# opencb/hpg-variant

Hardware: AMD Instinct MI355X
Metric: variants/s chi2 assoc (higher is better)
Workload: dtype u8

## Files before the change

hpg-variant_amd/csrc/hpgv_capi.hip:

```cpp
#include "hpgv_internal.h"
#include <cstdlib>

extern "C" {

const char *hpgv_version(void) { return "hpgv-mi355x 0.1 (gfx950)"; }

int hpgv_device_count(void) {
    int n = 0;
    if (hipGetDeviceCount(&n) != hipSuccess) return -1;
    return n;
}

const char *hpgv_last_error(const hpgv_ctx *ctx) { return ctx ? ctx->err.c_str() : g_create_error.c_str(); }

static void read_environment(hpgv_ctx *ctx) {
    auto num = [](const char *name, long lo, long hi, long *out) { const char *e = getenv(name); if (e && *e) { long v = atol(e); *out = v < lo ? lo : v > hi ? hi : v; } };
    num("HPGV_BATCH_COPY", 0, 1, &ctx->batch_copy);
    num("HPGV_BATCH_FUSED", 0, 1, &ctx->batch_fused);
    num("HPGV_STATS_ALL2", 0, 1, &ctx->stats_all2);
    num("HPGV_ASSOC_ROWS", 0, 1, &ctx->assoc_rows);
    num("HPGV_PINNED_NONCOHERENT", 0, 1, &ctx->pinned_noncoherent);
    num("HPGV_VMM_TRACE", 0, 1, &ctx->vmm_trace);
    num("HPGV_DECODE_TILES", 0, 1, &ctx->decode_tiles);
#ifdef HPGV_ABLATION
// ... 69 lines not shown
    g->device = g->members[0]->device;
    *out = g;
    return HPGV_OK;
}

int hpgv_group_size(const hpgv_ctx *ctx) { return !ctx ? 0 : (is_group(ctx) ? (int)ctx->members.size() : 1); }

hpgv_ctx *hpgv_group_member(hpgv_ctx *ctx, int i) {
    if (!ctx) return nullptr;
    if (!is_group(ctx)) return i == 0 ? ctx : nullptr;
    return (i >= 0 && i < (int)ctx->members.size()) ? ctx->members[(size_t)i] : nullptr;
}

int hpgv_member_device(const hpgv_ctx *ctx, int i) {
    if (!ctx) return -1;
    if (!is_group(ctx)) return i == 0 ? ctx->device : -1;
    return (i >= 0 && i < (int)ctx->members.size()) ? ctx->members[(size_t)i]->device : -1;
}

}
namespace {
void grow_release(hpgv_ctx::GrowRange &r) {
    size_t off = 0;
    for (size_t i = 0; i < r.pieces.size(); ++i) { (void)hipMemUnmap(r.base + off, r.sizes[i]); (void)hipMemRelease(r.pieces[i]); off += r.sizes[i]; }
    if (r.base) (void)hipMemAddressFree(r.base, r.reserved);
    r = hpgv_ctx::GrowRange();
}
}
extern "C" {

void hpgv_destroy(hpgv_ctx *ctx) {
    if (!ctx) return;
    if (is_group(ctx)) {
        hpgv_group_release(ctx);
        for (hpgv_ctx *m : ctx->members) { m->parent = nullptr; hpgv_destroy(m); }
        ctx->members.clear();
        delete ctx;
        return;
    }
    DeviceGuard g(ctx->device);
    (void)hipDeviceSynchronize();
    if (ctx->d_mendel_male) (void)hipFree(ctx->d_mendel_male);
    for (DevBuf *b : {&ctx->d_sg_chunks, &ctx->d_group_of_col, &ctx->d_cond, &ctx->d_perm, &ctx->d_strata, &ctx->d_cmh_tables, &ctx->d_cov, &ctx->d_lin, &ctx->d_linperm, &ctx->d_linperm_rows, &ctx->d_flips, &ctx->d_flip_tail, &ctx->d_thr, &ctx->assoc.d_cols, &ctx->tdt.d_cols,
                      &ctx->stats.d_cols, &ctx->sgroups.d_cols, &ctx->mendel.d_cols}) b->release();
    ctx->tdt_plan.release();
    if (ctx->d_lf_base) (void)hipFree(ctx->d_lf_base);
    if (ctx->d_sink) (void)hipFree(ctx->d_sink);
    if (ctx->d_crc_tab) (void)hipFree(ctx->d_crc_tab);
    for (auto *t : ctx->tok_scratch) {
        for (DevBuf *b : {&t->blocks, &t->line_off, &t->extra}) b->release();
        delete t;
    }
    ctx->tok_scratch.clear();
    for (auto &r : ctx->grow) grow_release(r);
    ctx->grow.clear();
    hpgv_epi_release(ctx->epi);
    for (Slot *s : ctx->slots) {
        s->release();
        if (s->stream) (void)hipStreamDestroy(s->stream);
        delete s;
    }
    for (int i = 0; i < 4; ++i) if (ctx->ev[i]) (void)hipEventDestroy(ctx->ev[i]);
    delete ctx;
}

#ifdef HPGV_ABLATION
#define HPGV_SHIPPED_ONLY(ok, what)
#else
#define HPGV_SHIPPED_ONLY(ok, what) if (!(ok)) return fail(ctx, HPGV_ERR_UNSUPPORTED, what ": that form is an ablation build's (-DHPGV_ABLATION, tools/build_ablation.py)");
#endif

int hpgv_set_option(hpgv_ctx *ctx, const char *key, long value) {
    if (is_group(ctx) && key && !strcmp(key, "group_self_exchange")) { ctx->group_self_exchange = value ? 1 : 0; return HPGV_OK; }
    if (is_group(ctx) && key && !strcmp(key, "group_fake_ranks")) {
        if (value < 0 || value > 65536) return fail(ctx, HPGV_ERR_INVALID, "group_fake_ranks must be 0 (ranks by distinct device) or the number of members that share rank 0");
        std::lock_guard<std::mutex> lk(ctx->mu);
        if (ctx->grp) return fail(ctx, HPGV_ERR_STATE, "group_fake_ranks must be set before the group's communicator exists (hpgv_group_comm_init, the first group call)");
        ctx->group_fake_ranks = value;
        return HPGV_OK;
    }
    GROUP_ALL(ctx, hpgv_set_option(m_, key, value))
    if (!ctx || !key) return HPGV_ERR_INVALID;
    if (!strcmp(key, "row_align")) {
        if (value < 16 || (value & (value - 1))) return fail(ctx, HPGV_ERR_INVALID, "row_align must be a power of two >= 16");
        if (ctx->assoc.set || ctx->tdt.set || ctx->stats.set)
            return fail(ctx, HPGV_ERR_STATE, "row_align must be set before the cohort");
        ctx->row_align = value;
    } else if (!strcmp(key, "row_pad")) {
        if (value < 0 || value % 16 || value > 65536) return fail(ctx, HPGV_ERR_INVALID, "row_pad must be a multiple of 16 in [0, 65536]");
        if (ctx->assoc.set || ctx->tdt.set || ctx->stats.set)
            return fail(ctx, HPGV_ERR_STATE, "row_pad must be set before the cohort");
        ctx->row_pad = value;
    } else if (!strcmp(key, "variants_per_wave")) {
        if (value < 1 || value > 1024) return fail(ctx, HPGV_ERR_INVALID, "variants_per_wave out of range");
        ctx->vpw = value;
    } else if (!strcmp(key, "nontemporal")) {
        HPGV_SHIPPED_ONLY(value != 0, "nontemporal = 0")
        ctx->nontemporal = value ? 1 : 0;
    } else if (!strcmp(key, "profile")) {
        ctx->profile = value ? 1 : 0;
    } else if (!strcmp(key, "scan_unroll")) {
        if (value != 4 && value != 8 && value != 10 && value != 12 && value != 16)
            return fail(ctx, HPGV_ERR_INVALID, "scan_unroll must be one of 4, 8, 10, 12, 16");
        HPGV_SHIPPED_ONLY(value == 4, "scan_unroll other than 4")
        ctx->scan_unroll = value;
    } else if (!strcmp(key, "pipeline")) {
        HPGV_SHIPPED_ONLY(value != 0, "pipeline = 0")
        ctx->pipeline = value ? 1 : 0;
    } else if (!strcmp(key, "fisher_cut_exp")) {
        if (value < 12 || value > 300) return fail(ctx, HPGV_ERR_INVALID, "fisher_cut_exp must be in [12, 300]");
        ctx->fisher_cut_exp = value;
    } else if (!strcmp(key, "epi_complete")) {
        ctx->epi_complete = value ? 1 : 0;
    } else if (!strcmp(key, "epi_triples_mfma")) {
        ctx->epi_triples_mfma = value ? 1 : 0;
    } else if (!strcmp(key, "epi_pairs_mfma")) {
        ctx->epi_pairs_mfma = value ? 1 : 0;
    } else if (!strcmp(key, "epi_wide")) {
        if (value < 0 || value > 2) return fail(ctx, HPGV_ERR_INVALID, "epi_wide must be 0 (the packed kernels' limits), 1 (the wide kernel where the shape needs it) or 2 (the wide kernel for every listed-combination launch)");
        ctx->epi_wide = value;
    } else if (!strcmp(key, "epi_triples_1pass")) {
        if (value < 0 || value > 2) return fail(ctx, HPGV_ERR_INVALID, "epi_triples_1pass must be 0 (two passes), 1 (the cells nine at a time) or 2 (one pass, one wave per SIMD)");
        HPGV_SHIPPED_ONLY(value != 2, "epi_triples_1pass = 2")
        ctx->epi_triples_1pass = value;
    } else if (!strcmp(key, "scan_lds")) {
        if (value < 0 || value > 160 * 1024) return fail(ctx, HPGV_ERR_INVALID, "scan_lds must be in [0, 163840]");
        ctx->scan_lds = value;
    } else if (!strcmp(key, "batch_copy")) {
        ctx->batch_copy = value ? 1 : 0;
    } else if (!strcmp(key, "inflate_wave")) {
        if (value < 0 || value > 4) return fail(ctx, HPGV_ERR_INVALID, "inflate_wave must be 0 (lane per block), 1 (by the number of blocks), 2 (wave per block), 4 (wave per block, several symbols per round) or 3 (lane per block, symbol tables in LDS)");
        HPGV_SHIPPED_ONLY(value == 1 || value == 4, "inflate_wave other than 1 / 4 (a wave per block, several symbols per round)")
        ctx->inflate_wave = value;
    } else if (!strcmp(key, "tokenizer_tiles")) {
        if (value < 0 || value > 2) return fail(ctx, HPGV_ERR_INVALID, "tokenizer_tiles must be 2 (one sweep), 1 (two sweeps) or 0 (line by line)");
        HPGV_SHIPPED_ONLY(value == 1, "tokenizer_tiles other than 1 (two sweeps)")
        ctx->tokenizer_tiles = value;
    } else if (!strcmp(key, "fisher_width")) {
        if (value != 64 && value != 32 && value != 16 && value != 8) return fail(ctx, HPGV_ERR_INVALID, "fisher_width must be 64, 32, 16 or 8");
        HPGV_SHIPPED_ONLY(value == 16, "fisher_width other than 16")
        ctx->fisher_width = value;
    } else if (!strcmp(key, "batch_fused")) {
        ctx->batch_fused = value ? 1 : 0;
    } else if (!strcmp(key, "pipe_waves")) {
        if (value != 4 && value != 6 && value != 8) return fail(ctx, HPGV_ERR_INVALID, "pipe_waves must be 4, 6 or 8");
        HPGV_SHIPPED_ONLY(value == 4, "pipe_waves other than 4")
        ctx->pipe_waves = value;
    } else if (!strcmp(key, "persistent")) {
        HPGV_SHIPPED_ONLY(value == 0, "persistent = 1")
        ctx->persistent = value ? 1 : 0;
    } else if (!strcmp(key, "part_aligned_loads")) {
        HPGV_SHIPPED_ONLY(value == 0, "part_aligned_loads = 1")
        ctx->part_aligned = value ? 1 : 0;
    } else if (!strcmp(key, "pca_apply_vector")) {
        HPGV_SHIPPED_ONLY(value == 0, "pca_apply_vector = 1")
        ctx->pca_apply_vector = value ? 1 : 0;
    } else if (!strcmp(key, "blocks_per_cu")) {
        if (value < 1 || value > 8) return fail(ctx, HPGV_ERR_INVALID, "blocks_per_cu must be in 1..8");
        ctx->blocks_per_cu = value;
    } else {
        return fail(ctx, HPGV_ERR_INVALID, "unknown option '%s'", key);
    }
    return HPGV_OK;
}


int hpgv_set_cohort(hpgv_ctx *ctx, const uint8_t *condition, int n_samples) {
    HPGV_ABI_TRY
    GROUP_ALL(ctx, hpgv_set_cohort(m_, condition, n_samples))
    if (!ctx) return HPGV_ERR_INVALID;
    if (!condition || n_samples < 0) return fail(ctx, HPGV_ERR_INVALID, "bad cohort arguments");
    DeviceGuard g(ctx->device);
    int nA = 0, nU = 0;
    for (int j = 0; j < n_samples; ++j) {
        if (condition[j] == HPGV_COND_AFFECTED) nA++;
        else if (condition[j] == HPGV_COND_UNAFFECTED) nU++;
    }
    size_t segA = round_up((size_t)nA, 16), segU = round_up((size_t)nU, 16);
    size_t pitch = round_up(segA + segU, (size_t)ctx->row_align) + (size_t)ctx->row_pad;
    if (pitch == 0) pitch = (size_t)ctx->row_align;
    if (!pitch_supported(pitch)) return fail(ctx, HPGV_ERR_UNSUPPORTED, "cohort of %d samples exceeds the row-length limit", n_samples);
    Layout &L = ctx->assoc;
    ctx->n_perms = ctx->perm_rows = 0;
    ctx->n_covar = 0;
    ctx->n_strata = ctx->strata_rows = 0;
    ctx->has_pheno = false; ctx->lin_y.clear(); ctx->lin_cov.clear();
    ctx->n_linperms = 0;
    L.n_samples = n_samples;
    L.pitch = pitch;
    L.col_of_pos.assign(pitch, -1);
    size_t a = 0, u = segA;
    for (int j = 0; j < n_samples; ++j) {
        if (condition[j] == HPGV_COND_AFFECTED) L.col_of_pos[a++] = j;
        else if (condition[j] == HPGV_COND_UNAFFECTED) L.col_of_pos[u++] = j;
    }
    ctx->nA = nA; ctx->nU = nU; ctx->chunksA = (int)(segA / 16);
    {
        std::vector<uint8_t> cond(round_up((size_t)n_samples, 16) + 16, (uint8_t)HPGV_COND_OTHER);
        for (int j = 0; j < n_samples; ++j) cond[(size_t)j] = condition[j] == HPGV_COND_AFFECTED ? 1 : condition[j] == HPGV_COND_UNAFFECTED ? 0 : 2;
        HIPCHK(ctx, ctx->d_cond.reserve(cond.size()));
        HIPCHK(ctx, hipMemcpy(ctx->d_cond.p, cond.data(), cond.size(), hipMemcpyHostToDevice));
    }
    return upload_layout(ctx, L);
    HPGV_ABI_CATCH(ctx)
}

int hpgv_assoc_layout(const hpgv_ctx *ctx, int *n_affected, int *n_unaffected, size_t *pitch) {
    ctx = first_member(ctx);
    if (!ctx) return HPGV_ERR_INVALID;
    if (!ctx->assoc.set) return fail(ctx, HPGV_ERR_STATE, "hpgv_set_cohort has not been called");
    if (n_affected) *n_affected = ctx->nA;
    if (n_unaffected) *n_unaffected = ctx->nU;
    if (pitch) *pitch = ctx->assoc.pitch;
    return HPGV_OK;
}

int hpgv_set_logfact(hpgv_ctx *ctx, const double *table, size_t n) {
    GROUP_ALL(ctx, hpgv_set_logfact(m_, table, n))
    if (!ctx) return HPGV_ERR_INVALID;
    if (!table || n == 0) return fail(ctx, HPGV_ERR_INVALID, "empty log-factorial table");
    DeviceGuard g(ctx->device);
    ctx->n_lf = 0;
    if (ctx->cap_lf < n) {
        if (ctx->d_lf_base) { (void)hipFree(ctx->d_lf_base); ctx->d_lf_base = nullptr; ctx->d_lf = nullptr; ctx->cap_lf = 0; }
        HIPCHK(ctx, hipMalloc(&ctx->d_lf_base, (n + 4) * sizeof(double)));
        HIPCHK(ctx, hipMemset(ctx->d_lf_base, 0, (n + 4) * sizeof(double)));
        ctx->d_lf = ctx->d_lf_base + 2;
        ctx->cap_lf = n;
    }
    HIPCHK(ctx, hipMemcpy(ctx->d_lf, table, n * sizeof(double), hipMemcpyHostToDevice));
    ctx->n_lf = n;
    return HPGV_OK;
}

int hpgv_set_stats_cohort(hpgv_ctx *ctx, int n_samples) {
    HPGV_ABI_TRY
    GROUP_ALL(ctx, hpgv_set_stats_cohort(m_, n_samples))
    if (!ctx) return HPGV_ERR_INVALID;
    if (n_samples < 0) return fail(ctx, HPGV_ERR_INVALID, "negative n_samples");
    DeviceGuard g(ctx->device);
    size_t pitch = round_up(round_up((size_t)n_samples, 16), (size_t)ctx->row_align);
    if (pitch == 0) pitch = (size_t)ctx->row_align;
    if (!pitch_supported(pitch)) return fail(ctx, HPGV_ERR_UNSUPPORTED, "cohort of %d samples exceeds the row-length limit", n_samples);
    Layout &L = ctx->stats;
    L.n_samples = n_samples;
    L.pitch = pitch;
    L.col_of_pos.assign(pitch, -1);
    for (int j = 0; j < n_samples; ++j) L.col_of_pos[j] = j;
    return upload_layout(ctx, L);
    HPGV_ABI_CATCH(ctx)
}

int hpgv_set_stats_groups(hpgv_ctx *ctx, const int32_t *group_of_sample, int n_samples, int n_groups) {
    HPGV_ABI_TRY
    GROUP_ALL(ctx, hpgv_set_stats_groups(m_, group_of_sample, n_samples, n_groups))
    if (!ctx) return HPGV_ERR_INVALID;
    if (n_samples < 0 || n_groups < 1 || n_groups > 4096 || (n_samples > 0 && !group_of_sample))
        return fail(ctx, HPGV_ERR_INVALID, "bad stats group arguments");
    DeviceGuard g(ctx->device);
    std::vector<int> size((size_t)n_groups, 0);
    for (int j = 0; j < n_samples; ++j) {
        if (group_of_sample[j] >= n_groups) return fail(ctx, HPGV_ERR_INVALID, "group %d of sample %d out of range", group_of_sample[j], j);
        if (group_of_sample[j] >= 0) size[(size_t)group_of_sample[j]]++;
    }
    std::vector<uint32_t> off((size_t)n_groups, 0);
    size_t used = 0;
    for (int k = 0; k < n_groups; ++k) { off[(size_t)k] = (uint32_t)used; used += round_up((size_t)size[(size_t)k], 16); }
    size_t pitch = round_up(used, (size_t)ctx->row_align) + (size_t)ctx->row_pad;
    if (pitch == 0) pitch = (size_t)ctx->row_align;
    if (!pitch_supported(pitch)) return fail(ctx, HPGV_ERR_UNSUPPORTED, "cohort of %d samples exceeds the row-length limit", n_samples);
    Layout &L = ctx->sgroups;
    L.n_samples = n_samples;
    L.pitch = pitch;
    L.col_of_pos.assign(pitch, -1);
    std::vector<size_t> fill(off.begin(), off.end());
    for (int j = 0; j < n_samples; ++j)
        if (group_of_sample[j] >= 0) L.col_of_pos[fill[(size_t)group_of_sample[j]]++] = j;
    ctx->sg_off = off;
    ctx->sg_size = size;
    {
// ... 369 lines not shown
```

hpg-variant_amd/csrc/hpgv_internal.h:

```cpp
#pragma once
#include "../../include/hpgv.h"
#include "hpgv_kernels.h"
#include "hpgv_tdt_stats_kernels.h"
#include "hpgv_epi_kernels.h"

#include <hip/hip_runtime.h>
#include <cctype>

#include <algorithm>
#include <atomic>
#include <cmath>
#include <cstdarg>
#include <cstdio>
#include <cstring>
#include <functional>
#include <mutex>
#include <new>
#include <string>
#include <vector>

namespace { thread_local std::string g_create_error; }

struct DevBuf {
    void *p = nullptr;
// ... 105 lines not shown
    uint32_t rev_off = 0;
    hpgv_epi_rank_info rank_info{};
    uint32_t *d_marg = nullptr;
    bool complete = false;
    hpgv::EpiChunk *d_chunks = nullptr;
    uint32_t *d_chunk_cls = nullptr;
    hpgv::EpiFold *d_folds = nullptr;
    uint32_t *d_group_w0 = nullptr;
    std::vector<int32_t> group_size;
    DevBuf cand;
    unsigned *d_cand_count = nullptr;
    unsigned cand_cap = 0;
    double *d_thr = nullptr;
    DevBuf tile_base;
};

struct hpgv_ctx {
    std::vector<hpgv_ctx *> members;
    hpgv_ctx *parent = nullptr;
    struct GroupState *grp = nullptr;
    long group_self_exchange = 0;
    long group_fake_ranks = 0;
    std::atomic<unsigned> deal_next{0};
    std::atomic<int> in_flight{0};
    int device = 0;
    mutable std::string err;
    std::mutex mu;
    long row_align = 16;
    long row_pad = 0;
    long vpw = 2;
    long nontemporal = 1;
    long profile = 0;
    std::mutex alias_mu;
    std::vector<std::pair<const char *, const char *>> text_alias;
    struct TextTiles { const char *d_text, *d_base; const void *d_tiles; uint64_t n_tiles; };
    std::vector<TextTiles> text_tiles;
    struct TextHeld { const char *host_text; Slot *slot; const char *d_text; const unsigned long long *d_line_off; int n_lines; };
    std::vector<TextHeld> text_held;
    long part_aligned = 0;
    long pca_apply_vector = 0;
    long scan_unroll = 4;
    long persistent = 0;
    long blocks_per_cu = 8;
    long pipeline = 1;
    long pipe_waves = 4;
    long fisher_cut_exp = 22;
    long epi_complete = 1;
    long epi_pairs_mfma = 1;
    long epi_triples_mfma = 1;
    long epi_wide = 0;
    long epi_triples_1pass = 1;
    long scan_lds = 0;
    long fisher_width = 16;
    long inflate_wave = 1;
    long tokenizer_tiles = 1;
    long batch_copy = 0;
    long batch_fused = 1;
    long batch_lds_max = 65536;
    long stats_all2 = 1;
    long assoc_rows = 1;
    long pinned_noncoherent = 0;
    long vmm_trace = 0;
    long decode_tiles = 1;
#ifdef HPGV_ABLATION
    long stats_rows = 0, stats_bs = 0, stats_debug = 0;
    long fisher_lds = 0;
    long inflate_lds_pad = 0, inflate_wave_wgs = 0, inflate_lane_wgs = 0;
#endif
    int n_cus = 256;
    Layout assoc;
    int nA = 0, nU = 0, chunksA = 0;
    DevBuf d_cond;
    DevBuf d_perm;
    int n_perms = 0, perm_rows = 0;
    DevBuf d_strata;
    int n_strata = 0, strata_rows = 0;
    DevBuf d_cmh_tables;
    DevBuf d_cov;
    int n_covar = 0;
    std::vector<double> lin_y, lin_cov;
    bool has_pheno = false;
    DevBuf d_lin;
    DevBuf d_linperm;
    int n_linperms = 0;
    DevBuf d_linperm_rows;
    Layout tdt;
    hpgv::TdtPlan tdt_plan;
    DevBuf d_flips;
    int n_flips = 0, flip_rows = 0, flip_pitch = 0;
    int tdt_families = 0;
    DevBuf d_flip_tail;
    Layout stats;
    Layout sgroups;
    std::vector<uint32_t> sg_off;
    std::vector<int> sg_size;
    DevBuf d_sg_chunks;
    DevBuf d_group_of_col;
    bool all_grouped = false;
    Layout mendel;
    int mendel_trios = 0, mendel_pchunks = 0;
    hpgv::MendelLuts mendel_luts{};
    uint8_t *d_mendel_male = nullptr;
    double *d_lf = nullptr;
    double *d_lf_base = nullptr;
    size_t n_lf = 0;
    size_t cap_lf = 0;
    DevBuf d_thr;
    hipEvent_t ev[4] = {nullptr, nullptr, nullptr, nullptr};
    bool have_scan_ev = false, have_stats_ev = false;
    std::vector<Slot *> slots;
    uint32_t *d_sink = nullptr;
    uint32_t *d_crc_tab = nullptr;
    struct TokScratch {
        hipStream_t stream = nullptr;
        DevBuf blocks, line_off, extra;
    };
    std::mutex tok_mu;
    std::vector<TokScratch *> tok_scratch;
    struct GrowRange { char *base = nullptr; size_t reserved = 0, committed = 0; std::vector<hipMemGenericAllocationHandle_t> pieces; std::vector<size_t> sizes; };
    std::vector<GrowRange> grow;
    double filt_min_maf = -1.0, filt_max_missing = -1.0;
    long filt_max_mendel = -1;
    double filt_min_dom = -1.0, filt_min_rec = -1.0;
    std::mutex epi_mu;
    EpiState epi;
};

namespace {

[[maybe_unused]] int fail(const hpgv_ctx *ctx, int code, const char *fmt, ...) {
    char buf[512];
    va_list ap;
    va_start(ap, fmt);
    vsnprintf(buf, sizeof buf, fmt, ap);
    va_end(ap);
    if (ctx) {
        ctx->err = buf;
        if (ctx->parent) {
            std::lock_guard<std::mutex> lk(ctx->parent->mu);
            ctx->parent->err = buf;
        }
    } else g_create_error = buf;
    return code;
}

#define HPGV_ABI_TRY try {
#define HPGV_ABI_CATCH(ctx)                                                                         \
    } catch (const std::bad_alloc &) { return fail(ctx, HPGV_ERR_NOMEM, "out of host memory"); }     \
      catch (...) { return fail(ctx, HPGV_ERR_INVALID, "unexpected C++ exception inside the engine"); }

inline bool is_group(const hpgv_ctx *c) { return c && !c->members.empty(); }
inline hpgv_ctx *first_member(hpgv_ctx *c) { return is_group(c) ? c->members[0] : c; }
inline const hpgv_ctx *first_member(const hpgv_ctx *c) { return is_group(c) ? c->members[0] : c; }
struct Dealt {
    hpgv_ctx *m;
    explicit Dealt(hpgv_ctx *g) {
        const unsigned n = (unsigned)g->members.size(), start = g->deal_next.fetch_add(1u, std::memory_order_relaxed) % n;
        m = g->members[start];
        int best = m->in_flight.load(std::memory_order_relaxed);
        for (unsigned k = 1; k < n && best > 0; ++k) {
            hpgv_ctx *c = g->members[(start + k) % n];
            const int f = c->in_flight.load(std::memory_order_relaxed);
            if (f < best) { best = f; m = c; }
        }
        m->in_flight.fetch_add(1, std::memory_order_relaxed);
    }
    ~Dealt() { m->in_flight.fetch_sub(1, std::memory_order_relaxed); }
};
#define GROUP_ALL(ctx, CALL)                                                                \
    if (is_group(ctx)) {                                                                    \
        for (hpgv_ctx *m_ : (ctx)->members) { const int rc_ = CALL; if (rc_) return rc_; }  \
// ... 199 lines not shown
```

hpg-variant_amd/csrc/hpgv_kernels.h:

```cpp
#pragma once
#include <hip/hip_runtime.h>
#include <stdint.h>

namespace hpgv {

__device__ __forceinline__ uint32_t nib_nonzero(uint32_t x) {
    uint32_t y = x | (x << 1);
    y = y | (y << 2);
    return y & 0x88888888u;
}
__device__ __forceinline__ uint32_t nib_not_f(uint32_t x) { return nib_nonzero(~x); }

__device__ __forceinline__ int wave_sum(int v) {
    v += __builtin_amdgcn_update_dpp(0, v, 0xB1, 0xF, 0xF, true);
    v += __builtin_amdgcn_update_dpp(0, v, 0x4E, 0xF, 0xF, true);
    v += __builtin_amdgcn_update_dpp(0, v, 0x141, 0xF, 0xF, true);
    v += __builtin_amdgcn_update_dpp(0, v, 0x140, 0xF, 0xF, true);
    return __builtin_amdgcn_readlane(v, 0) + __builtin_amdgcn_readlane(v, 16) +
           __builtin_amdgcn_readlane(v, 32) + __builtin_amdgcn_readlane(v, 48);
}

template <bool NT>
__device__ __forceinline__ uint4 load16(const uint4 *p);
template <bool NT>
// ... 219 lines not shown
    const int i = blockIdx.x * blockDim.x + threadIdx.x;
    if (i >= n) return;
    const int4 c4 = counts[i];
    const int a = c4.x, c = c4.y, b = c4.z, d = c4.w;
    const double x = assoc_chisq_value(a, c, b, d);
    odds[i] = assoc_odds(a, c, b, d);
    chisq[i] = x;
    pval[i] = chisq_p_value(x);
}

__device__ __forceinline__ double wave_sum_f64(double v) {
#pragma unroll
    for (int off = 32; off > 0; off >>= 1) v += __shfl_xor(v, off);
    return v;
}
__device__ __forceinline__ double wave_max_f64(double v) {
#pragma unroll
    for (int off = 32; off > 0; off >>= 1) { const double o = __shfl_xor(v, off); v = o > v ? o : v; }
    return v;
}

__device__ const double k_exp2_j64[64] = {
    0x1.0000000000000p+0, 0x1.02c9a3e778061p+0, 0x1.059b0d3158574p+0, 0x1.0874518759bc8p+0,
    0x1.0b5586cf9890fp+0, 0x1.0e3ec32d3d1a2p+0, 0x1.11301d0125b51p+0, 0x1.1429aaea92de0p+0,
    0x1.172b83c7d517bp+0, 0x1.1a35beb6fcb75p+0, 0x1.1d4873168b9aap+0, 0x1.2063b88628cd6p+0,
    0x1.2387a6e756238p+0, 0x1.26b4565e27cddp+0, 0x1.29e9df51fdee1p+0, 0x1.2d285a6e4030bp+0,
    0x1.306fe0a31b715p+0, 0x1.33c08b26416ffp+0, 0x1.371a7373aa9cbp+0, 0x1.3a7db34e59ff7p+0,
    0x1.3dea64c123422p+0, 0x1.4160a21f72e2ap+0, 0x1.44e086061892dp+0, 0x1.486a2b5c13cd0p+0,
    0x1.4bfdad5362a27p+0, 0x1.4f9b2769d2ca7p+0, 0x1.5342b569d4f82p+0, 0x1.56f4736b527dap+0,
    0x1.5ab07dd485429p+0, 0x1.5e76f15ad2148p+0, 0x1.6247eb03a5585p+0, 0x1.6623882552225p+0,
    0x1.6a09e667f3bcdp+0, 0x1.6dfb23c651a2fp+0, 0x1.71f75e8ec5f74p+0, 0x1.75feb564267c9p+0,
    0x1.7a11473eb0187p+0, 0x1.7e2f336cf4e62p+0, 0x1.82589994cce13p+0, 0x1.868d99b4492edp+0,
    0x1.8ace5422aa0dbp+0, 0x1.8f1ae99157736p+0, 0x1.93737b0cdc5e5p+0, 0x1.97d829fde4e50p+0,
    0x1.9c49182a3f090p+0, 0x1.a0c667b5de565p+0, 0x1.a5503b23e255dp+0, 0x1.a9e6b5579fdbfp+0,
    0x1.ae89f995ad3adp+0, 0x1.b33a2b84f15fbp+0, 0x1.b7f76f2fb5e47p+0, 0x1.bcc1e904bc1d2p+0,
    0x1.c199bdd85529cp+0, 0x1.c67f12e57d14bp+0, 0x1.cb720dcef9069p+0, 0x1.d072d4a07897cp+0,
    0x1.d5818dcfba487p+0, 0x1.da9e603db3285p+0, 0x1.dfc97337b9b5fp+0, 0x1.e502ee78b3ff6p+0,
    0x1.ea4afa2a490dap+0, 0x1.efa1bee615a27p+0, 0x1.f50765b6e4540p+0, 0x1.fa7c1819e90d8p+0,
};
__device__ __forceinline__ double fisher_exp(double e, const double *tab ) {
    const double kf = __builtin_rint(e * 0x1.71547652b82fep+6);
    double r = __builtin_fma(-kf, 0x1.62e42fe000000p-7, e);
    r = __builtin_fma(-kf, 0x1.f473de6af278fp-36, r);
    const int ki = (int)kf;
    const double tj = tab[ki & 63];
    double q = __builtin_fma(r, 1.0 / 120.0, 1.0 / 24.0);
    q = __builtin_fma(r, q, 1.0 / 6.0);
    q = __builtin_fma(r, q, 0.5);
    q = __builtin_fma(r * r, q, r);
    const double y = __builtin_fma(tj, q, tj);
    return e < -1100.0 ? 0.0 : __builtin_ldexp(y, ki >> 6);
}

struct FisherTab {
    const double *lf; const double *xt ; double konst; int r1, c1, d0;
    __device__ __forceinline__ double at(uint32_t byte_off) const { return *reinterpret_cast<const double *>(reinterpret_cast<const char *>(lf) + byte_off); }
    __device__ __forceinline__ double e(int x) const {
        const uint32_t x8 = (uint32_t)x << 3;
        return konst - at(x8) - at(((uint32_t)r1 << 3) - x8) - at(((uint32_t)c1 << 3) - x8) - at(((uint32_t)d0 << 3) + x8);
    }
    __device__ __forceinline__ double p(int x) const { return fisher_exp(e(x), xt); }
    __device__ __forceinline__ void e2(int x, double *e0, double *e1) const {
        const char *b = reinterpret_cast<const char *>(lf) - 16;
        double2 q0, q1, q2, q3;
        __builtin_memcpy(&q0, b + ((uint32_t)(x + 2) << 3), 16);
        __builtin_memcpy(&q1, b + ((uint32_t)(r1 - x + 1) << 3), 16);
        __builtin_memcpy(&q2, b + ((uint32_t)(c1 - x + 1) << 3), 16);
        __builtin_memcpy(&q3, b + ((uint32_t)(d0 + x + 2) << 3), 16);
        *e0 = konst - q0.x - q1.y - q2.y - q3.x;
        *e1 = konst - q0.y - q1.x - q2.x - q3.y;
    }
};

template <int W> __device__ __forceinline__ int sub_lane(int lane) { return lane & (W - 1); }
template <int W> __device__ __forceinline__ uint64_t sub_ballot(bool pred, int lane) {
    const uint64_t b = __ballot(pred);
    if constexpr (W == 64) { (void)lane; return b; }
    else return (b >> (lane & ~(W - 1))) & ((1ull << W) - 1ull);
}
template <int W> __device__ __forceinline__ double sub_sum_f64(double v) {
#pragma unroll
    for (int off = W / 2; off > 0; off >>= 1) v += __shfl_xor(v, off);
    return v;
}
template <int W> __device__ __forceinline__ double sub_first_f64(double v, int lane) { return __shfl(v, lane & ~(W - 1)); }

template <int W>
__device__ __forceinline__ void fisher_boundaries(const FisherTab &T, double thr , int L1, int R1, int L2, int R2, int lane,
                                                  int *xL, int *xR) {
    const int sl = sub_lane<W>(lane);
    while (R1 - L1 > W || R2 - L2 > W) {
        const bool go1 = R1 - L1 > W, go2 = R2 - L2 > W;
        const int step1 = (R1 - L1 + W - 1) / W, step2 = (R2 - L2 + W - 1) / W;
        const int x1 = L1 + sl * step1, x2 = L2 + sl * step2;
        const double v1 = (go1 && x1 < R1) ? T.e(x1) : 0.0;
        const double v2 = (go2 && x2 < R2) ? T.e(x2) : 0.0;
        if (go1) {
            const int j = __builtin_popcountll(sub_ballot<W>(x1 < R1 && v1 <= thr, lane));
            const int xj = L1 + j * step1;
            const int nL = (j == 0) ? L1 : L1 + (j - 1) * step1 + 1, nR = (j == W || xj >= R1) ? R1 : xj;
            L1 = nL; R1 = nR;
        }
        if (go2) {
            const int j = __builtin_popcountll(sub_ballot<W>(x2 < R2 && v2 > thr, lane));
            const int xj = L2 + j * step2;
            const int nL = (j == 0) ? L2 : L2 + (j - 1) * step2 + 1, nR = (j == W || xj >= R2) ? R2 : xj;
            L2 = nL; R2 = nR;
        }
    }
    const int x1 = L1 + sl, x2 = L2 + sl;
    const double v1 = x1 < R1 ? T.e(x1) : 0.0, v2 = x2 < R2 ? T.e(x2) : 0.0;
    *xL = L1 + __builtin_popcountll(sub_ballot<W>(x1 < R1 && v1 <= thr, lane));
    *xR = L2 + __builtin_popcountll(sub_ballot<W>(x2 < R2 && v2 > thr, lane));
}

template <int W>
__device__ __forceinline__ double fisher_tails(const FisherTab &T, int xL, int xR, int lo, int hi, int lane, double rel_cut) {
    const int sl = sub_lane<W>(lane);
    double partL = 0.0, partR = 0.0, cutL = 0.0, cutR = 0.0;
    bool onL = true, onR = true;
    for (int k = 0; onL || onR; ++k) {
        const int firstL = xL - 1 - 2 * W * k, firstR = xR + 2 * W * k;
        if (firstL < lo) onL = false;
// ... 45 lines not shown
    T.lf = lf; T.xt = exp_tab; T.r1 = r1; T.c1 = c1; T.d0 = r2 - c1;
    T.konst = lf[r1] + lf[r2] + lf[c1] + lf[nn - c1] - lf[nn];
    const double thr = T.e(a) + 9.9999995000000333e-08;
    double sum;
    if (hi - lo < 8 * W) {
        double part = 0.0;
        for (int x = lo + sl; x <= hi; x += W) {
            const double ex = T.e(x);
            if (ex <= thr) part += fisher_exp(ex, exp_tab);
        }
        sum = sub_sum_f64<W>(part);
    } else {
        const double prod = (double)(r1 + 1) * (double)(c1 + 1), den = (double)(nn + 2);
        double md = __builtin_floor(prod / den);
        const double rem = __builtin_fma(-md, den, prod);
        md += rem >= den ? 1.0 : (rem < 0.0 ? -1.0 : 0.0);
        int mode = (int)md;
        mode = mode < lo ? lo : (mode > hi ? hi : mode);
        int L1 = lo, R1 = mode + 1, L2 = mode + 1, R2 = hi + 1, xL, xR;
        if (fisher_boundary_windows<W>(T, thr, mode, a, lane, &L1, &R1, &L2, &R2)) { xL = L1; xR = L2; }
        else fisher_boundaries<W>(T, thr, L1, R1, L2, R2, lane, &xL, &xR);
        sum = fisher_tails<W>(T, xL, xR, lo, hi, lane, rel_cut);
    }
    return sum > 1.0 ? 1.0 : sum;
}

__device__ __forceinline__ double fisher_wave(int a, int b, int c, int d, const double *__restrict__ lf,
                                              const double *exp_tab , double rel_cut, int lane) {
    return fisher_sub<64>(a, b, c, d, lf, exp_tab, rel_cut, lane);
}

template <int W>
__global__ __launch_bounds__(256) void k_assoc_fisher(const int4 *__restrict__ counts, int n,
                                                      const double *__restrict__ lf,
                                                      double *__restrict__ odds,
                                                      double *__restrict__ pval, double rel_cut) {
    __shared__ double exp_tab[64];
    if (threadIdx.x < 64) exp_tab[threadIdx.x] = k_exp2_j64[threadIdx.x];
    __syncthreads();
    const int lane = threadIdx.x & 63;
    constexpr int PER_WAVE = 64 / W;
    const long wave = (long)blockIdx.x * (blockDim.x >> 6) + (threadIdx.x >> 6);
    const long v = wave * PER_WAVE + lane / W;
    if (v >= n) return;
    const int4 c4 = counts[v];
    const int a = c4.x, b = c4.y, c = c4.z, d = c4.w;
    const double p = fisher_sub<W>(a, b, c, d, lf, exp_tab, rel_cut, lane);
    if (sub_lane<W>(lane) == 0) {
        odds[v] = assoc_odds(a, b, c, d);
        pval[v] = p;
    }
}

__host__ __device__ __forceinline__ uint64_t splitmix64(uint64_t x) {
    x ^= x >> 30; x *= 0xbf58476d1ce4e5b9ULL;
    x ^= x >> 27; x *= 0x94d049bb133111ebULL;
    x ^= x >> 31;
    return x;
}
#define HPGV_SYNTH_SEED 0x4850475631ULL

static __global__ void k_synth_thresholds(uint64_t v0, int n, uint32_t *__restrict__ thr) {
    const int i = blockIdx.x * blockDim.x + threadIdx.x;
    if (i >= n) return;
    const uint64_t v = v0 + (uint64_t)i;
    const uint64_t h = splitmix64(HPGV_SYNTH_SEED ^ 0xA11E1EULL ^ v);
    const double u = (double)(h >> 11) * (1.0 / 9007199254740992.0);
    const double q = 0.05 + 0.45 * u;
    const uint32_t t_miss = 167772u;
    const double rest = (double)(16777216u - t_miss);
    const double omq = 1.0 - q;
    const double p00 = omq * omq;
    const double p01 = 2.0 * q * omq;
    const uint32_t t00 = t_miss + (uint32_t)floor(p00 * rest);
    const uint32_t t01 = t00 + (uint32_t)floor(p01 * rest);
    thr[3 * i + 0] = t_miss; thr[3 * i + 1] = t00; thr[3 * i + 2] = t01;
}

__device__ __forceinline__ uint32_t synth_gt(uint64_t vterm, uint64_t s, uint32_t tm, uint32_t t0,
                                             uint32_t t1) {
    const uint32_t r = (uint32_t)(splitmix64(vterm + s) >> 40);
    return (r < tm) ? 0xFFu : (r < t0) ? 0x00u : (r < t1) ? 0x01u : 0x11u;
}

enum { RECODE_NONE = 0, RECODE_TDT = 1, RECODE_STATS = 2, RECODE_MENDEL = 3, RECODE_EPI = 4 };

constexpr uint32_t TDT_F_UNUSABLE = 0x80u, TDT_M_UNUSABLE = 0x20u;
constexpr uint32_t TDT_C_INVALID = 4u;

__host__ __device__ __forceinline__ uint32_t tdt_parent_class(uint32_t g, uint32_t unusable) {
    const uint32_t a1 = g >> 4, a2 = g & 0xFu;
    if (a1 == 0xFu || a2 == 0xFu) return unusable;
    if (a1 && !a2) return unusable;
    if (!a1 && !a2) return 0u;
    if (!a1) return 1u;
    return (a1 == a2) ? 2u : 3u;
}
__host__ __device__ __forceinline__ uint32_t tdt_child_class(uint32_t g) {
    const uint32_t a1 = g >> 4, a2 = g & 0xFu;
    if (a1 == 0xFu || a2 == 0xFu) return TDT_C_INVALID;
    if (!a1 && !a2) return 0u;
    if (!a1) return 1u;
    if (!a2) return 2u;
    return 3u;
}
__host__ __device__ __forceinline__ uint32_t stats_flags(uint32_t g) {
// ... 139 lines not shown
```

hpg-variant_amd/csrc/hpgv_scan_capi.hip:

```cpp
#include "hpgv_internal.h"
#include <type_traits>
#include "hpgv_inherit_kernels.h"

namespace {

unsigned scan_blocks(const hpgv_ctx *ctx, int n_variants) {
    const long waves = ((long)n_variants + ctx->vpw - 1) / ctx->vpw;
    return (unsigned)((waves + 3) / 4);
}

const char *const kAligned16 = "device buffers must be 16-byte aligned";
int scan_checks(hpgv_ctx *ctx, int n_variants, const void *d_gt, const void *d_out, uintptr_t out_mask, const char *align_text, bool *go) {
    *go = false;
    if (n_variants < 0 || (n_variants > 0 && (!d_gt || !d_out))) return fail(ctx, HPGV_ERR_INVALID, "bad scan arguments");
    if (n_variants == 0) return HPGV_OK;
    if (((uintptr_t)d_gt & 15) || ((uintptr_t)d_out & out_mask)) return fail(ctx, HPGV_ERR_INVALID, "%s", align_text);
    *go = true;
    return HPGV_OK;
}

template <typename F>
void launch_nt(const hpgv_ctx *ctx, F &&f) {
    if (ctx->nontemporal) f(std::true_type{}); else f(std::false_type{});
}
// ... 152 lines not shown
    do {                                                                                         \
        if (ctx->pipe_waves == 8) { HPGV_LAUNCH_PIPE(NT, U, 8); }                                \
        else if (ctx->pipe_waves == 6) { HPGV_LAUNCH_PIPE(NT, U, 6); }                           \
        else { HPGV_LAUNCH_PIPE(NT, U, 4); }                                                     \
    } while (0)
    if (ctx->pipeline && !ctx->persistent)
        return launch_profiled(ctx, st, 0, [&] {
            if (ctx->nontemporal) {
                if (ctx->scan_unroll <= 4) HPGV_PIPE_W(true, 4); else HPGV_PIPE_W(true, 5);
            } else {
                if (ctx->scan_unroll <= 4) HPGV_PIPE_W(false, 4); else HPGV_PIPE_W(false, 5);
            }
        });
    return launch_profiled(ctx, st, 0, [&] {
        if (ctx->nontemporal) {
            if (ctx->persistent) { HPGV_DISPATCH_U(true, true) } else { HPGV_DISPATCH_U(true, false) }
        } else {
            if (ctx->persistent) { HPGV_DISPATCH_U(false, true) } else { HPGV_DISPATCH_U(false, false) }
        }
    });
#undef HPGV_DISPATCH_U
#undef HPGV_PIPE_W
#undef HPGV_LAUNCH_ASSOC
#endif
#undef HPGV_LAUNCH_PIPE
}

int hpgv_assoc_chisq_dev(hpgv_ctx *ctx, const int32_t *d_counts, int n_variants, double *d_odds,
                         double *d_chisq, double *d_p, void *stream) {
    ctx = first_member(ctx);
    if (!ctx) return HPGV_ERR_INVALID;
    if (n_variants < 0 || (n_variants > 0 && (!d_counts || !d_odds || !d_chisq || !d_p)))
        return fail(ctx, HPGV_ERR_INVALID, "bad chisq arguments");
    if (n_variants == 0) return HPGV_OK;
    DeviceGuard g(ctx->device);
    hipStream_t st = (hipStream_t)stream;
    return launch_profiled(ctx, st, 1, [&] {
        hipLaunchKernelGGL(hpgv::k_assoc_chisq, dim3((n_variants + 255) / 256), dim3(256), 0, st,
                           (const int4 *)d_counts, n_variants, d_odds, d_chisq, d_p);
    });
}

int hpgv_assoc_fisher_dev(hpgv_ctx *ctx, const int32_t *d_counts, int n_variants, double *d_odds,
                          double *d_p, void *stream) {
    ctx = first_member(ctx);
    if (!ctx) return HPGV_ERR_INVALID;
    if (n_variants < 0 || (n_variants > 0 && (!d_counts || !d_odds || !d_p)))
        return fail(ctx, HPGV_ERR_INVALID, "bad fisher arguments");
    if (const int rc = logfact_check(ctx)) return rc;
    if (n_variants == 0) return HPGV_OK;
    DeviceGuard g(ctx->device);
    hipStream_t st = (hipStream_t)stream;
    const double cut = pow(10.0, -(double)ctx->fisher_cut_exp);
    return launch_profiled(ctx, st, 1, [&] {
        const long per_block = 4 * (64 / ctx->fisher_width);
        const unsigned blocks = (unsigned)(((long)n_variants + per_block - 1) / per_block);
#ifdef HPGV_ABLATION
        const unsigned pad = (unsigned)ctx->fisher_lds;
        if (ctx->fisher_width == 64)
            hipLaunchKernelGGL(hpgv::k_assoc_fisher<64>, dim3(blocks), dim3(256), pad, st, (const int4 *)d_counts, n_variants, ctx->d_lf, d_odds, d_p, cut);
        else if (ctx->fisher_width == 8)
            hipLaunchKernelGGL(hpgv::k_assoc_fisher<8>, dim3(blocks), dim3(256), pad, st, (const int4 *)d_counts, n_variants, ctx->d_lf, d_odds, d_p, cut);
        else if (ctx->fisher_width == 32)
            hipLaunchKernelGGL(hpgv::k_assoc_fisher<32>, dim3(blocks), dim3(256), pad, st, (const int4 *)d_counts, n_variants, ctx->d_lf, d_odds, d_p, cut);
        else
#else
        const unsigned pad = 0u;
#endif
            hipLaunchKernelGGL(hpgv::k_assoc_fisher<16>, dim3(blocks), dim3(256), pad, st, (const int4 *)d_counts, n_variants, ctx->d_lf, d_odds, d_p, cut);
    });
}


int hpgv_tdt_scan_dev(hpgv_ctx *ctx, const uint8_t *d_gt, int n_variants, const uint8_t *d_is_x,
                      int32_t *d_tu, void *stream) {
    ctx = first_member(ctx);
    if (!ctx) return HPGV_ERR_INVALID;
    if (!ctx->tdt.set) return fail(ctx, HPGV_ERR_STATE, "hpgv_set_families has not been called");
    bool go;
    if (const int rc = scan_checks(ctx, n_variants, d_gt, d_tu, 7, "device buffers must be aligned", &go); rc || !go) return rc;
    DeviceGuard g(ctx->device);
    hipStream_t st = (hipStream_t)stream;
    return launch_profiled(ctx, st, 0, [&] {
        ctx->tdt_plan.launch_scan(d_gt, ctx->tdt.pitch, n_variants, d_is_x, (int2 *)d_tu,
                                  (int)ctx->vpw, ctx->nontemporal != 0, st);
    });
}

int hpgv_tdt_stats_dev(hpgv_ctx *ctx, const int32_t *d_tu, int n_variants, double *d_odds,
                       double *d_chisq, double *d_p, void *stream) {
    ctx = first_member(ctx);
    if (!ctx) return HPGV_ERR_INVALID;
    if (n_variants < 0 || (n_variants > 0 && (!d_tu || !d_odds || !d_chisq || !d_p)))
        return fail(ctx, HPGV_ERR_INVALID, "bad tdt stats arguments");
    if (n_variants == 0) return HPGV_OK;
    DeviceGuard g(ctx->device);
    hipStream_t st = (hipStream_t)stream;
    return launch_profiled(ctx, st, 1, [&] {
        hipLaunchKernelGGL(hpgv::k_tdt_stats, dim3((n_variants + 255) / 256), dim3(256), 0, st,
                           (const int2 *)d_tu, n_variants, d_odds, d_chisq, d_p);
    });
}


static int stats_scan(hpgv_ctx *ctx, const Layout &L, const uint8_t *d_gt, int n_variants, uint32_t off, int chunks, size_t lds,
                      int32_t *d_counts8, hipStream_t st) {
// ... 198 lines not shown
```

Before: 136.1 million.

## Split Fisher exact test into plan, scan and load-balanced sum kernels

For large Fisher calls, a plan kernel locates each variant's tail ranges with Newton steps and galloping search, then counts 32-term chunks. A prefix scan over those counts lets a persistent sum kernel give every 16-lane group an equal share of chunks. This is meant to remove the load imbalance from variants with very different tail lengths. It adds two extra launches, a per-stream scratch buffer, and a larger zero pad on the log-factorial table.

New measurement: 135.8 million, median of 2. No clear change (-0.2%).

```diff
diff --git a/hpg-variant_amd/csrc/hpgv_capi.hip b/hpg-variant_amd/csrc/hpgv_capi.hip
--- a/hpg-variant_amd/csrc/hpgv_capi.hip
+++ b/hpg-variant_amd/csrc/hpgv_capi.hip
@@ -145,6 +145,8 @@
         delete t;
     }
     ctx->tok_scratch.clear();
+    for (auto *t : ctx->fisher_scratch) { t->buf.release(); delete t; }
+    ctx->fisher_scratch.clear();
     for (auto &r : ctx->grow) grow_release(r);
     ctx->grow.clear();
     hpgv_epi_release(ctx->epi);
@@ -233,6 +235,9 @@
         if (value != 64 && value != 32 && value != 16 && value != 8) return fail(ctx, HPGV_ERR_INVALID, "fisher_width must be 64, 32, 16 or 8");
         HPGV_SHIPPED_ONLY(value == 16, "fisher_width other than 16")
         ctx->fisher_width = value;
+    } else if (!strcmp(key, "fisher_dense_min")) {
+        if (value < 0) return fail(ctx, HPGV_ERR_INVALID, "fisher_dense_min must be 0 (every call in two phases) or a number of variants");
+        ctx->fisher_dense_min = value;
     } else if (!strcmp(key, "batch_fused")) {
         ctx->batch_fused = value ? 1 : 0;
     } else if (!strcmp(key, "pipe_waves")) {
@@ -316,9 +321,9 @@
     ctx->n_lf = 0;
     if (ctx->cap_lf < n) {
         if (ctx->d_lf_base) { (void)hipFree(ctx->d_lf_base); ctx->d_lf_base = nullptr; ctx->d_lf = nullptr; ctx->cap_lf = 0; }
-        HIPCHK(ctx, hipMalloc(&ctx->d_lf_base, (n + 4) * sizeof(double)));
-        HIPCHK(ctx, hipMemset(ctx->d_lf_base, 0, (n + 4) * sizeof(double)));
-        ctx->d_lf = ctx->d_lf_base + 2;
+        HIPCHK(ctx, hipMalloc(&ctx->d_lf_base, (n + 2 * hpgv::FISHER_LF_PAD) * sizeof(double)));
+        HIPCHK(ctx, hipMemset(ctx->d_lf_base, 0, (n + 2 * hpgv::FISHER_LF_PAD) * sizeof(double)));
+        ctx->d_lf = ctx->d_lf_base + hpgv::FISHER_LF_PAD;
         ctx->cap_lf = n;
     }
     HIPCHK(ctx, hipMemcpy(ctx->d_lf, table, n * sizeof(double), hipMemcpyHostToDevice));
diff --git a/hpg-variant_amd/csrc/hpgv_internal.h b/hpg-variant_amd/csrc/hpgv_internal.h
--- a/hpg-variant_amd/csrc/hpgv_internal.h
+++ b/hpg-variant_amd/csrc/hpgv_internal.h
@@ -181,6 +181,7 @@
     long epi_triples_1pass = 1;
     long scan_lds = 0;
     long fisher_width = 16;
+    long fisher_dense_min = 524288;
     long inflate_wave = 1;
     long tokenizer_tiles = 1;
     long batch_copy = 0;
@@ -246,6 +247,12 @@
     };
     std::mutex tok_mu;
     std::vector<TokScratch *> tok_scratch;
+    struct FisherScratch {
+        hipStream_t stream = nullptr;
+        DevBuf buf;
+    };
+    std::vector<FisherScratch *> fisher_scratch;
+    int fisher_sum_blocks = 0;
     struct GrowRange { char *base = nullptr; size_t reserved = 0, committed = 0; std::vector<hipMemGenericAllocationHandle_t> pieces; std::vector<size_t> sizes; };
     std::vector<GrowRange> grow;
     double filt_min_maf = -1.0, filt_max_missing = -1.0;
diff --git a/hpg-variant_amd/csrc/hpgv_kernels.h b/hpg-variant_amd/csrc/hpgv_kernels.h
--- a/hpg-variant_amd/csrc/hpgv_kernels.h
+++ b/hpg-variant_amd/csrc/hpgv_kernels.h
@@ -295,6 +295,7 @@
     return e < -1100.0 ? 0.0 : __builtin_ldexp(y, ki >> 6);
 }
 
+constexpr int FISHER_LF_PAD = 40;
 struct FisherTab {
     const double *lf; const double *xt ; double konst; int r1, c1, d0;
     __device__ __forceinline__ double at(uint32_t byte_off) const { return *reinterpret_cast<const double *>(reinterpret_cast<const char *>(lf) + byte_off); }
@@ -303,15 +304,24 @@
         return konst - at(x8) - at(((uint32_t)r1 << 3) - x8) - at(((uint32_t)c1 << 3) - x8) - at(((uint32_t)d0 << 3) + x8);
     }
     __device__ __forceinline__ double p(int x) const { return fisher_exp(e(x), xt); }
-    __device__ __forceinline__ void e2(int x, double *e0, double *e1) const {
-        const char *b = reinterpret_cast<const char *>(lf) - 16;
+    __device__ __forceinline__ void e2_at(uint32_t o0, uint32_t o1, uint32_t o2, uint32_t o3, double *e0, double *e1) const {
+        const char *b = reinterpret_cast<const char *>(lf) - 8 * FISHER_LF_PAD;
         double2 q0, q1, q2, q3;
-        __builtin_memcpy(&q0, b + ((uint32_t)(x + 2) << 3), 16);
-        __builtin_memcpy(&q1, b + ((uint32_t)(r1 - x + 1) << 3), 16);
-        __builtin_memcpy(&q2, b + ((uint32_t)(c1 - x + 1) << 3), 16);
-        __builtin_memcpy(&q3, b + ((uint32_t)(d0 + x + 2) << 3), 16);
+        __builtin_memcpy(&q0, b + o0, 16);
+        __builtin_memcpy(&q1, b + o1, 16);
+        __builtin_memcpy(&q2, b + o2, 16);
+        __builtin_memcpy(&q3, b + o3, 16);
         *e0 = konst - q0.x - q1.y - q2.y - q3.x;
         *e1 = konst - q0.y - q1.x - q2.x - q3.y;
+    }
+    __device__ __forceinline__ void offsets(int x, uint32_t *o0, uint32_t *o1, uint32_t *o2, uint32_t *o3) const {
+        *o0 = (uint32_t)(x + FISHER_LF_PAD) << 3; *o1 = (uint32_t)(r1 - x - 1 + FISHER_LF_PAD) << 3;
+        *o2 = (uint32_t)(c1 - x - 1 + FISHER_LF_PAD) << 3; *o3 = (uint32_t)(d0 + x + FISHER_LF_PAD) << 3;
+    }
+    __device__ __forceinline__ void e2(int x, double *e0, double *e1) const {
+        uint32_t o0, o1, o2, o3;
+        offsets(x, &o0, &o1, &o2, &o3);
+        e2_at(o0, o1, o2, o3, e0, e1);
     }
 };
 
@@ -463,6 +473,214 @@
     }
 }
 
+struct FisherPlan { double konst, thr; int pos1, end1, pos2, end2; };
+constexpr int FISHER_CHUNK = 32;
+constexpr int FISHER_PLAN_BLOCK = 256;
+__host__ __device__ constexpr unsigned fisher_chunks(int pos1, int end1, int pos2, int end2) {
+    const unsigned c = (unsigned)(end1 - pos1 + FISHER_CHUNK - 1) / FISHER_CHUNK + (unsigned)(end2 - pos2 + FISHER_CHUNK - 1) / FISHER_CHUNK;
+    return c ? c : 1u;
+}
+
+template <typename P>
+__device__ __forceinline__ int fisher_count_true(P pred, int N, int guess) {
+    if (N <= 0) return 0;
+    int L = 0, R = N, s = 1;
+    const int g = guess < 0 ? 0 : (guess > N - 1 ? N - 1 : guess);
+    if (pred(g)) {
+        L = g + 1;
+        while (L < R) { const int x = (R - L > s) ? L + s - 1 : R - 1; if (pred(x)) { L = x + 1; s *= 4; } else { R = x; break; } }
+    } else {
+        R = g;
+        while (L < R) { const int x = (R - L > s) ? R - s : L; if (!pred(x)) { R = x; s *= 4; } else { L = x + 1; break; } }
+    }
+    while (L < R) { const int m = L + ((R - L) >> 1); if (pred(m)) L = m + 1; else R = m; }
+    return L;
+}
+__device__ __forceinline__ int fisher_newton(const FisherTab &T, int x, double target, int xmin, int xmax) {
+    x = x < xmin ? xmin : (x > xmax ? xmax : x);
+    const float num = (float)(T.r1 - x) * (float)(T.c1 - x), den = (float)(x + 1) * (float)(T.d0 + x + 1);
+    const float dx = (float)(target - T.e(x)) / __logf(num / den);
+    if (!(__builtin_fabsf(dx) < 1e6f)) return x;
+    const int y = x + (int)__builtin_rintf(dx);
+    return y < xmin ? xmin : (y > xmax ? xmax : y);
+}
+
+__device__ __forceinline__ int fisher_tail_end(const FisherTab &T, int x, double cutline, int xmin, int xmax, int dir) {
+    x = x < xmin ? xmin : (x > xmax ? xmax : x);
+#pragma unroll 1
+    for (int k = 0; k < 2; ++k) {
+        const float num = (float)(T.r1 - x) * (float)(T.c1 - x), den = (float)(x + 1) * (float)(T.d0 + x + 1);
+        const float dx = (float)(cutline - T.e(x)) / __logf(num / den);
+        if (!(__builtin_fabsf(dx) < 1e6f)) return dir > 0 ? xmax : xmin;
+        const int y = x + (int)(dir > 0 ? __builtin_ceilf(dx) : __builtin_floorf(dx)) + dir;
+        const int moved = y > x ? y - x : x - y;
+        x = y < xmin ? xmin : (y > xmax ? xmax : y);
+        if (moved <= 8) break;
+    }
+    return x;
+}
+
+static __global__ __launch_bounds__(FISHER_PLAN_BLOCK) void k_assoc_fisher_plan(const int4 *__restrict__ counts, int n, const double *__restrict__ lf,
+                                                                          double ln_cut, FisherPlan *__restrict__ plan,
+                                                                          double *__restrict__ odds, uint32_t *__restrict__ local_start,
+                                                                          uint32_t *__restrict__ block_sum) {
+    __shared__ uint32_t wave_tot[FISHER_PLAN_BLOCK / 64];
+    const long v = (long)blockIdx.x * FISHER_PLAN_BLOCK + threadIdx.x;
+    uint32_t chunks = 0;
+    if (v < n) {
+        const int4 c4 = counts[v];
+        const int a = c4.x, b = c4.y, c = c4.z, d = c4.w;
+        const int r1 = a + b, r2 = c + d, c1 = a + c, nn = r1 + r2;
+        const int lo = (c1 - r2) > 0 ? (c1 - r2) : 0;
+        const int hi = r1 < c1 ? r1 : c1;
+        FisherTab T;
+        T.lf = lf; T.xt = nullptr; T.r1 = r1; T.c1 = c1; T.d0 = r2 - c1;
+        T.konst = lf[r1] + lf[r2] + lf[c1] + lf[nn - c1] - lf[nn];
+        const double thr = T.e(a) + 9.9999995000000333e-08;
+        FisherPlan P;
+        P.konst = T.konst;
+        if (hi - lo < 8 * 16) {
+            P.thr = thr; P.pos1 = lo; P.end1 = hi + 1; P.pos2 = P.end2 = lo;
+        } else {
+            const double prod = (double)(r1 + 1) * (double)(c1 + 1), den = (double)(nn + 2);
+            double md = __builtin_floor(prod / den);
+            const double rem = __builtin_fma(-md, den, prod);
+            md += rem >= den ? 1.0 : (rem < 0.0 ? -1.0 : 0.0);
+            int mode = (int)md;
+            mode = mode < lo ? lo : (mode > hi ? hi : mode);
+            const bool left = a <= mode;
+            int gL = left ? a + 1 : 2 * mode - a + 1, gR = left ? 2 * mode - a : a;
+            if (left) { if (hi > mode) gR = fisher_newton(T, gR, thr, mode + 1, hi); }
+            else gL = fisher_newton(T, gL, thr, lo, mode);
+            double e_firstL = 0.0, e_firstR = 0.0;
+            const int xL = lo + fisher_count_true([&](int i) { const double ex = T.e(lo + i); const bool in = ex <= thr; if (in) e_firstL = ex; return in; },
+                                                  mode + 1 - lo, gL - lo);
+            const int xR = mode + 1 + fisher_count_true([&](int i) { const double ex = T.e(mode + 1 + i); const bool out = ex > thr; if (!out) e_firstR = ex; return out; },
+                                                        hi - mode, gR - (mode + 1));
+            const float fn = (float)nn, var2 = 2.0f * (float)r1 * (float)r2 / fn * (float)c1 / fn * (float)(nn - c1) / (fn > 1.0f ? fn - 1.0f : 1.0f);
+            int lenL = 0, lenR = 0;
+            if (xL > lo) {
+                const int first = xL - 1;
+                const float z = (float)(mode - first);
+                const int end = fisher_tail_end(T, first - (int)(__builtin_sqrtf(z * z - var2 * (float)ln_cut) - __builtin_fabsf(z)), e_firstL + ln_cut, lo, first, -1);
+                lenL = first - end + 1;
+            }
+            if (xR <= hi) {
+                const float z = (float)(xR - mode);
+                const int end = fisher_tail_end(T, xR + (int)(__builtin_sqrtf(z * z - var2 * (float)ln_cut) - __builtin_fabsf(z)), e_firstR + ln_cut, xR, hi, 1);
+                lenR = end - xR + 1;
+            }
+            P.thr = __builtin_huge_val(); P.pos1 = xL - lenL; P.end1 = xL; P.pos2 = xR; P.end2 = xR + lenR;
+        }
+        plan[v] = P;
+        odds[v] = assoc_odds(a, b, c, d);
+        chunks = fisher_chunks(P.pos1, P.end1, P.pos2, P.end2);
+    }
+    const int lane = threadIdx.x & 63, wave = threadIdx.x >> 6;
+    uint32_t incl = chunks;
+#pragma unroll
+    for (int off = 1; off < 64; off <<= 1) { const uint32_t o = __shfl_up(incl, off); if (lane >= off) incl += o; }
+    if (lane == 63) wave_tot[wave] = incl;
+    __syncthreads();
+    uint32_t before = 0, all = 0;
+#pragma unroll
+    for (int w = 0; w < FISHER_PLAN_BLOCK / 64; ++w) { const uint32_t t = wave_tot[w]; all += t; if (w < wave) before += t; }
+    if (v < n) local_start[v] = before + incl - chunks;
+    if (threadIdx.x == 0) block_sum[blockIdx.x] = all;
+}
+
+static __global__ __launch_bounds__(1024) void k_assoc_fisher_offsets(const uint32_t *__restrict__ block_sum, int nb, unsigned long long *__restrict__ block_off) {
+    __shared__ unsigned long long s[1024];
+    const int tid = threadIdx.x, per = (nb + 1023) / 1024;
+    const long b0 = (long)tid * per, b1 = b0 + per < nb ? b0 + per : nb;
+    unsigned long long sum = 0;
+    for (long i = b0; i < b1; ++i) sum += block_sum[i];
+    s[tid] = sum;
+    __syncthreads();
+    for (int off = 1; off < 1024; off <<= 1) {
+        const unsigned long long t = tid >= off ? s[tid - off] : 0ull;
+        __syncthreads();
+        s[tid] += t;
+        __syncthreads();
+    }
+    unsigned long long run = s[tid] - sum;
+    for (long i = b0; i < b1; ++i) { block_off[i] = run; run += block_sum[i]; }
+    if (tid == 1023) block_off[nb] = s[1023];
+}
+
+__device__ __forceinline__ double row16_sum_f64(double v) {
+#define HPGV_ROW_STEP(ctrl)                                                                                  \
+    {                                                                                                        \
+        const int l_ = __builtin_amdgcn_update_dpp(0, __double2loint(v), ctrl, 0xF, 0xF, false);            \
+        const int h_ = __builtin_amdgcn_update_dpp(0, __double2hiint(v), ctrl, 0xF, 0xF, false);            \
+        v += __hiloint2double(h_, l_);                                                                       \
+    }
+    HPGV_ROW_STEP(0xB1)
+    HPGV_ROW_STEP(0x4E)
+    HPGV_ROW_STEP(0x141)
+    HPGV_ROW_STEP(0x140)
+#undef HPGV_ROW_STEP
+    return v;
+}
+
+static __global__ __launch_bounds__(256) void k_assoc_fisher_sum(const FisherPlan *__restrict__ plan, const int4 *__restrict__ counts,
+                                                                 const uint32_t *__restrict__ local_start,
+                                                                 const unsigned long long *__restrict__ block_off, int n,
+                                                                 const double *__restrict__ lf, double *__restrict__ pval) {
+    __shared__ double exp_tab[64];
+    if (threadIdx.x < 64) exp_tab[threadIdx.x] = k_exp2_j64[threadIdx.x];
+    __syncthreads();
+    const int sl2 = 2 * (threadIdx.x & 15);
+    const unsigned long long G = (unsigned long long)gridDim.x * 16, g = (unsigned long long)blockIdx.x * 16 + (threadIdx.x >> 4);
+    const unsigned long long total = block_off[(n + FISHER_PLAN_BLOCK - 1) / FISHER_PLAN_BLOCK], Q = (total + G - 1) / G;
+    auto start_of = [&](int vv) { return vv < n ? block_off[vv / FISHER_PLAN_BLOCK] + local_start[vv] : total; };
+    auto first_at = [&](unsigned long long key) {
+        int L = 0, R = n;
+        while (L < R) {
+            const int step = (R - L + 15) >> 4, m = L + (sl2 >> 1) * step;
+            const int j = __builtin_popcountll(sub_ballot<16>(m < R && start_of(m) < key, threadIdx.x & 63));
+            if (j == 0) R = L;
+            else { const int mj = L + j * step; R = (j < 16 && mj < R) ? mj : R; L = L + (j - 1) * step + 1; }
+        }
+        return L;
+    };
+    int v = first_at(g * Q);
+    const int vend = first_at((g + 1) * Q);
+    const int n_chunks = (int)(start_of(vend) - start_of(v));
+    FisherTab T;
+    T.lf = lf; T.xt = exp_tab;
+    double thr = 0.0, part = 0.0;
+    int rem = 0, pos2 = 0, end2 = 0;
+    uint32_t o0 = 0, o1 = 0, o2 = 0, o3 = 0;
+    auto range = [&](int pos, int end) { T.offsets(pos + sl2, &o0, &o1, &o2, &o3); rem = end - pos - sl2; };
+    auto load = [&](int vv) {
+        const FisherPlan P = plan[vv];
+        const int4 c4 = counts[vv];
+        T.konst = P.konst; T.r1 = c4.x + c4.y; T.c1 = c4.x + c4.z; T.d0 = c4.w - c4.x;
+        thr = P.thr; pos2 = P.pos2; end2 = P.end2;
+        if (P.pos1 < P.end1) range(P.pos1, P.end1);
+        else { range(pos2, end2); pos2 = end2; }
+    };
+    auto masked = [](double t, bool in) { return __hiloint2double(in ? __double2hiint(t) : (int)0xC09F4000, __double2loint(t)); };
+    if (n_chunks > 0) load(v);
+    for (int c = 0; c < n_chunks; ++c) {
+        double t0, t1;
+        T.e2_at(o0, o1, o2, o3, &t0, &t1);
+        const double e0 = masked(t0, rem > 0 && t0 <= thr), e1 = masked(t1, rem > 1 && t1 <= thr);
+        part += fisher_exp(e0, exp_tab) + fisher_exp(e1, exp_tab);
+        o0 += 8 * FISHER_CHUNK; o1 -= 8 * FISHER_CHUNK; o2 -= 8 * FISHER_CHUNK; o3 += 8 * FISHER_CHUNK; rem -= FISHER_CHUNK;
+        if (rem + sl2 <= 0) {
+            if (pos2 < end2) { range(pos2, end2); pos2 = end2; }
+            else {
+                const double sum = row16_sum_f64(part);
+                if (sl2 == 0) pval[v] = sum > 1.0 ? 1.0 : sum;
+                part = 0.0;
+                if (++v < vend) load(v);
+            }
+        }
+    }
+}
+
 __host__ __device__ __forceinline__ uint64_t splitmix64(uint64_t x) {
     x ^= x >> 30; x *= 0xbf58476d1ce4e5b9ULL;
     x ^= x >> 27; x *= 0x94d049bb133111ebULL;
diff --git a/hpg-variant_amd/csrc/hpgv_scan_capi.hip b/hpg-variant_amd/csrc/hpgv_scan_capi.hip
--- a/hpg-variant_amd/csrc/hpgv_scan_capi.hip
+++ b/hpg-variant_amd/csrc/hpgv_scan_capi.hip
@@ -228,6 +228,36 @@
     DeviceGuard g(ctx->device);
     hipStream_t st = (hipStream_t)stream;
     const double cut = pow(10.0, -(double)ctx->fisher_cut_exp);
+    if (ctx->fisher_width == 16 && n_variants >= ctx->fisher_dense_min) {
+        hpgv_ctx::FisherScratch *fs = nullptr;
+        {
+            std::lock_guard<std::mutex> lk(ctx->tok_mu);
+            for (auto *t : ctx->fisher_scratch) if (t->stream == st) fs = t;
+            if (!fs) { fs = new hpgv_ctx::FisherScratch(); fs->stream = st; ctx->fisher_scratch.push_back(fs); }
+            if (!ctx->fisher_sum_blocks) {
+                int per_cu = 0;
+                HIPCHK(ctx, hipOccupancyMaxActiveBlocksPerMultiprocessor(&per_cu, hpgv::k_assoc_fisher_sum, 256, 0));
+                ctx->fisher_sum_blocks = (per_cu > 0 ? per_cu : 1) * ctx->n_cus;
+            }
+        }
+        const size_t n = (size_t)n_variants, nb = (n + hpgv::FISHER_PLAN_BLOCK - 1) / hpgv::FISHER_PLAN_BLOCK;
+        const size_t off_boff = n * sizeof(hpgv::FisherPlan), off_local = off_boff + round_up((nb + 1) * sizeof(unsigned long long), 16),
+                     off_bsum = off_local + round_up(n * sizeof(uint32_t), 16), bytes = off_bsum + nb * sizeof(uint32_t);
+        HIPCHK(ctx, fs->buf.reserve_after_sync(st, bytes, bytes + bytes / 4));
+        char *base = fs->buf.as<char>();
+        hpgv::FisherPlan *plan = (hpgv::FisherPlan *)base;
+        unsigned long long *boff = (unsigned long long *)(base + off_boff);
+        uint32_t *local = (uint32_t *)(base + off_local), *bsum = (uint32_t *)(base + off_bsum);
+        const size_t want = (n + 15) / 16;
+        const unsigned sum_blocks = (unsigned)(want < (size_t)ctx->fisher_sum_blocks ? want : (size_t)ctx->fisher_sum_blocks);
+        return launch_profiled(ctx, st, 1, [&] {
+            hipLaunchKernelGGL(hpgv::k_assoc_fisher_plan, dim3((unsigned)nb), dim3(hpgv::FISHER_PLAN_BLOCK), 0, st, (const int4 *)d_counts, n_variants,
+                               ctx->d_lf, log(cut), plan, d_odds, local, bsum);
+            hipLaunchKernelGGL(hpgv::k_assoc_fisher_offsets, dim3(1), dim3(1024), 0, st, bsum, (int)nb, boff);
+            hipLaunchKernelGGL(hpgv::k_assoc_fisher_sum, dim3(sum_blocks), dim3(256), 0, st, plan, (const int4 *)d_counts, local, boff, n_variants,
+                               ctx->d_lf, d_p);
+        });
+    }
     return launch_profiled(ctx, st, 1, [&] {
         const long per_block = 4 * (64 / ctx->fisher_width);
         const unsigned blocks = (unsigned)(((long)n_variants + per_block - 1) / per_block);
```
